# t0saki/YOLO-Infer-pt

Hardware: AMD Instinct MI355X
Metric: images/sec at 640x640 batch32, v11_n (forward + on-device NMS) (higher is better)
Workload: dtype bf16; 1 GPU; yolo_v11_n eval forward + NMS, 640x640, 32 images per GPU per step; per_gpu_batch=32, global_batch=32, image_size=640, parallelism=dp1, nms=on-device, conf 0.001, iou 0.65, max_det 300

## Files before the change

### yolo-infer-pt_amd/csrc/c3k2.hip

```cpp
#include "common.h"
#include "dtypes.h"

namespace yh {

namespace {

typedef float f32x16 __attribute__((ext_vector_type(16)));

template <typename T> struct CMfma;
template <> struct CMfma<__bf16> {
    static __device__ __forceinline__ f32x16 step(const uint4& a, const uint4& b, const f32x16& c) {
        return __builtin_amdgcn_mfma_f32_32x32x16_bf16(__builtin_bit_cast(bf16x8, a), __builtin_bit_cast(bf16x8, b), c, 0,
                                                       0, 0);
    }
};
template <> struct CMfma<_Float16> {
    static __device__ __forceinline__ f32x16 step(const uint4& a, const uint4& b, const f32x16& c) {
        return __builtin_amdgcn_mfma_f32_32x32x16_f16(__builtin_bit_cast(f16x8, a), __builtin_bit_cast(f16x8, b), c, 0, 0,
                                                      0);
    }
};

constexpr int NWV = CSP_THREADS / 64;

__device__ __forceinline__ void cs_glds(const void* src, unsigned lds_addr) {
#if defined(__HIP_DEVICE_COMPILE__)
    unsigned keep;
    asm volatile("s_mov_b32 %0, m0\n\ts_mov_b32 m0, %2\n\ts_nop 0\n\tglobal_load_lds_dwordx4 %1, off\n\ts_mov_b32 m0, %0"
                 : "=&s"(keep) : "v"(src), "s"(lds_addr) : "memory");
#else
    (void)src; (void)lds_addr;
#endif
}
__device__ __forceinline__ void cs_barrier() { asm volatile("s_waitcnt lgkmcnt(0)\n\ts_barrier" ::: "memory"); }

__device__ __forceinline__ void cs_wait_vm(int n) {
    if (n >= 8) asm volatile("s_waitcnt vmcnt(8)" ::: "memory");
    else if (n >= 4) asm volatile("s_waitcnt vmcnt(4)" ::: "memory");
    else if (n >= 2) asm volatile("s_waitcnt vmcnt(2)" ::: "memory");
    else asm volatile("s_waitcnt vmcnt(0)" ::: "memory");
}

#ifdef YH_CSP_TRACE
constexpr int CS_TR = 12, CS_TR_TILES = 16, CS_TR_WG = 256, CS_TR_OPS = 4;
__device__ unsigned long long csp_trace_buf[CS_TR_OPS * CS_TR_WG * CS_TR_TILES * CS_TR];
#define CS_STAMP(k) do { if (trp) trp[k] = __builtin_amdgcn_s_memtime(); } while (0)
#else
#define CS_STAMP(k) do { } while (0)
#endif

__device__ __forceinline__ uint4 cs_rd(unsigned addr) {
#if defined(__HIP_DEVICE_COMPILE__)
    typedef __attribute__((address_space(3))) const uint4* lp;
    return *reinterpret_cast<lp>((size_t)addr);
#else
    (void)addr;
    return uint4{};
#endif
}
__device__ __forceinline__ void cs_wr(unsigned addr, uint4 v) {
#if defined(__HIP_DEVICE_COMPILE__)
    typedef __attribute__((address_space(3))) uint4* lp;
    *reinterpret_cast<lp>((size_t)addr) = v;
#else
    (void)addr; (void)v;
#endif
}
__device__ __forceinline__ float4 cs_rdf(unsigned addr) {
    const uint4 u = cs_rd(addr);
    return make_float4(__uint_as_float(u.x), __uint_as_float(u.y), __uint_as_float(u.z), __uint_as_float(u.w));
}

struct CsLayout {
    int w1, w2, w3, w4, b1, b2, b3, b4, prm;
};
__host__ __device__ constexpr CsLayout cs_layout(int ni, int nc, int no) {
    const int nh = (nc + 1) / 2, na3 = (nc + 1) / 2;
    CsLayout L{};
    L.w1 = 0;
    L.w2 = L.w1 + nc * ni * 1024;
    L.w3 = L.w2 + 9 * nc * 1024;
    L.w4 = L.w3 + na3 * 9 * nh * 1024;
    L.b1 = L.w4 + no * 3 * nc * 1024;
    L.b2 = L.b1 + 32 * nc * 4;
    L.b3 = L.b2 + 32 * 4;
    L.b4 = L.b3 + 32 * na3 * 4;
    L.prm = (L.b4 + 32 * no * 4 + 1023) & ~1023;
    return L;
}
struct CsTile {
    int lx, lt, lr, lc, total;
};
__host__ __device__ inline CsTile cs_tile(int TH, int TW, int ni, int nc, int no) {
    const int nh = (nc + 1) / 2;
    const CsLayout L = cs_layout(ni, nc, no);
    const int XP = (TH + 4) * (TW + 4), MP = (TH + 2) * (TW + 2), NP = TH * TW;
    CsTile t{};
    t.lx = L.prm;
    t.lt = t.lx + (ni ? ((XP * (16 * ni + 8) * 2 + 1023) & ~1023) : 0);
    t.lr = t.lt + XP * (32 * nc + 8) * 2;
    t.lc = t.lr + MP * (16 * nh + 8) * 2;
    t.total = t.lc + NP * (16 * nc + 8) * 2;
    return t;
}

template <typename T>
__device__ __forceinline__ void cs_act(const f32x16& acc, unsigned bias_addr, uint4 (&o)[2]) {
    float v[16];
#pragma unroll
    for (int q = 0; q < 4; ++q) {
        const float4 b = cs_rdf(bias_addr + 16 * q);
        v[4 * q] = acc[4 * q] + b.x;
        v[4 * q + 1] = acc[4 * q + 1] + b.y;
        v[4 * q + 2] = acc[4 * q + 2] + b.z;
        v[4 * q + 3] = acc[4 * q + 3] + b.w;
    }
    T t[16];
#pragma unroll
    for (int i = 0; i < 16; ++i) t[i] = fromf<T>(silu<T>(v[i]));
    o[0] = *reinterpret_cast<const uint4*>(&t[0]);
    o[1] = *reinterpret_cast<const uint4*>(&t[8]);
}

template <typename T>
__device__ __forceinline__ uint4 cs_act_half(const f32x16& acc, unsigned bias_addr, int hh) {
#if defined(__HIP_DEVICE_COMPILE__)
    float v[8];
#pragma unroll
    for (int e = 0; e < 8; ++e)
        v[e] = __uint_as_float(
            __builtin_amdgcn_permlane32_swap(__float_as_uint(acc[e]), __float_as_uint(acc[8 + e]), false, false)[0]);
    const float4 b0 = cs_rdf(bias_addr + 32 * hh), b1 = cs_rdf(bias_addr + 32 * hh + 16);
    v[0] += b0.x; v[1] += b0.y; v[2] += b0.z; v[3] += b0.w;
    v[4] += b1.x; v[5] += b1.y; v[6] += b1.z; v[7] += b1.w;
    T t[8];
#pragma unroll
    for (int i = 0; i < 8; ++i) {
        float p = silu<T>(v[i]);
        asm("" : "+v"(p));
        t[i] = fromf<T>(p);
    }
    return *reinterpret_cast<const uint4*>(&t[0]);
#else
    (void)acc; (void)bias_addr; (void)hh;
    return uint4{};
#endif
}

template <typename T, int NA, int NK, typename BAddr, typename Epi>
__device__ __forceinline__ void cs_phase(unsigned aimg, int npx, BAddr baddr, Epi epi) {
    const int lane = threadIdx.x & 63, wv = threadIdx.x >> 6, l32 = lane & 31;
    const int items = NA * ((npx + 31) >> 5);
    for (int i0 = wv; i0 < items; i0 += 2 * NWV) {
        const int i1 = i0 + NWV;
        const int a0 = i0 % NA, a1 = i1 % NA;
        const int p0 = (i0 / NA) * 32 + l32, p1 = (i1 / NA) * 32 + l32;
        const int c0 = p0 < npx ? p0 : npx - 1, c1 = p1 < npx ? p1 : npx - 1;
        const unsigned ai0 = aimg + (unsigned)(a0 * NK * 1024 + lane * 16);
        const unsigned ai1 = aimg + (unsigned)(a1 * NK * 1024 + lane * 16);
        f32x16 acc0, acc1;
#pragma unroll
        for (int e = 0; e < 16; ++e) { acc0[e] = 0.f; acc1[e] = 0.f; }
        if (i1 < items) {
#pragma unroll
            for (int k = 0; k < NK; ++k) {
                const uint4 f0 = cs_rd(ai0 + k * 1024), f1 = NA > 1 ? cs_rd(ai1 + k * 1024) : f0;
                const uint4 x0 = cs_rd(baddr(c0, k)), x1 = cs_rd(baddr(c1, k));
                acc0 = CMfma<T>::step(f0, x0, acc0);
                acc1 = CMfma<T>::step(f1, x1, acc1);
            }
            if (p0 < npx) epi(a0, p0, acc0);
            if (p1 < npx) epi(a1, p1, acc1);
        } else {
#pragma unroll
            for (int k = 0; k < NK; ++k) acc0 = CMfma<T>::step(cs_rd(ai0 + k * 1024), cs_rd(baddr(c0, k)), acc0);
            if (p0 < npx) epi(a0, p0, acc0);
        }
    }
}

#ifdef YH_CSP_TRACE
constexpr int cs_trace_op(int ni, int, int no) { return ni == 2 ? 0 : ni == 4 ? 1 : no == 2 ? 2 : 3; }
#endif

template <typename T, int NI, int NC, int NO>
__global__ __launch_bounds__(CSP_THREADS) void csp_fused(const CspArgs A) {
    constexpr int NH = (NC + 1) / 2, NA3 = (NC + 1) / 2;
    constexpr int SX = 16 * NI + 8, ST = 32 * NC + 8, SR = 16 * NH + 8, SC = 16 * NC + 8;
    constexpr CsLayout L = cs_layout(NI, NC, NO);
    extern __shared__ __attribute__((aligned(16))) char sm[];
    typedef __attribute__((address_space(3))) char* lds_c;
    const unsigned lds0 = (unsigned)(size_t)(lds_c)sm;
    const int TH = A.TH, TW = A.TW, XW = TW + 4, MW = TW + 2;
    const int XP = (TH + 4) * XW, MP = (TH + 2) * MW, NP = TH * TW;
    const CsTile G = cs_tile(TH, TW, NI, NC, NO);
    const unsigned LX = lds0 + G.lx, LT = lds0 + G.lt, LR = lds0 + G.lr, LC = lds0 + G.lc;
    const int lane = threadIdx.x & 63, hh = lane >> 5;
    const int wvu = __builtin_amdgcn_readfirstlane(threadIdx.x >> 6);
    const T* x = reinterpret_cast<const T*>(A.x);
    T* y = reinterpret_cast<T*>(A.y);

    {
        const char* prm = reinterpret_cast<const char*>(A.prm);
        for (int i0 = wvu * 64; i0 < L.prm / 16; i0 += CSP_THREADS) cs_glds(prm + (size_t)(i0 + lane) * 16, lds0 + i0 * 16);
    }
    constexpr bool TAIL = NI == 0;
    constexpr int NCH = TAIL ? 4 * NC : 2 * NI;
    constexpr int CPX = NCH + 1;
    const unsigned LD = TAIL ? LT : LX;
    auto load_x = [&](int t) {
        const int n = t / A.tiles, tix = t - n * A.tiles;
        const int ty = tix / A.ntw, tx = tix - ty * A.ntw;
        const int h0 = ty * TH - 2, w0 = tx * TW - 2;
        const int total = XP * CPX;
        for (int i0 = wvu * 64; i0 < total; i0 += CSP_THREADS) {
            const int q = i0 + lane;
            const int px = q / CPX, c = q - px * CPX;
            const int r = px / XW, cc = px - r * XW;
            const int gh = h0 + r, gw = w0 + cc;
            const bool ok = q < total && c < NCH && (unsigned)gh < (unsigned)A.H && (unsigned)gw < (unsigned)A.W;
            const void* src = ok ? (const void*)(x + (((long long)n * A.H + gh) * A.W + gw) * A.ldx + c * 8) : A.zero;
            cs_glds(src, LD + i0 * 16);
        }
    };
    const int t0 = xcd_remap(blockIdx.x, gridDim.x);
    if (t0 < A.ntiles) load_x(t0);

    const int p4_items = NO * ((NP + 31) >> 5);
    const int p4_stores = wvu < p4_items ? 2 * ((p4_items - wvu + NWV - 1) / NWV) : 0;
    int young = 0;
#ifdef YH_CSP_TRACE
    int trk = 0;
#endif
    for (int t = t0; t < A.ntiles; t += gridDim.x) {
        const int n = t / A.tiles, tix = t - n * A.tiles;
        const int ty = tix / A.ntw, tx = tix - ty * A.ntw;
        const int h0 = ty * TH, w0 = tx * TW;
#ifdef YH_CSP_TRACE
        unsigned long long* trp = nullptr;
        if (threadIdx.x == 0 && blockIdx.x < CS_TR_WG && trk < CS_TR_TILES) {
            trp = csp_trace_buf + ((size_t)(cs_trace_op(NI, NC, NO) * CS_TR_WG + blockIdx.x) * CS_TR_TILES + trk) * CS_TR;
            trp[10] = __builtin_amdgcn_s_memrealtime();
            trp[11] = (unsigned long long)TH | (unsigned long long)TW << 16 | (unsigned long long)(t + 1) << 32;
        }
        ++trk;
#endif
        CS_STAMP(0);
        cs_wait_vm(young);
        CS_STAMP(1);
        cs_barrier();
        CS_STAMP(2);

        if constexpr (!TAIL) {
        cs_phase<T, NC, NI>(
                lds0 + L.w1, XP,
                [&](int px, int k) { return LX + (unsigned)(px * SX + 16 * k + 8 * hh) * 2; },
                [&](int a, int px, const f32x16& acc) {
                    uint4 o[2];
                    cs_act<T>(acc, lds0 + L.b1 + (32 * a + 16 * hh) * 4, o);
                    const int r = px / XW, cc = px - r * XW;
                    const int gh = h0 - 2 + r, gw = w0 - 2 + cc;
                    if (!((unsigned)gh < (unsigned)A.H && (unsigned)gw < (unsigned)A.W)) o[0] = o[1] = make_uint4(0, 0, 0, 0);
                    const unsigned d = LT + (unsigned)(px * ST + 32 * a + 16 * hh) * 2;
                    cs_wr(d, o[0]);
                    cs_wr(d + 16, o[1]);
                });
        CS_STAMP(3);
        cs_barrier();
        CS_STAMP(4);
        if (t + (int)gridDim.x < A.ntiles) load_x(t + gridDim.x);
        }

        cs_phase<T, 1, 9 * NC>(
            lds0 + L.w2, MP,
            [&](int px, int k) {
                const int cb = k / 9, tap = k - 9 * (k / 9), kh = tap / 3, kw = tap - 3 * (tap / 3);
                const int r = px / MW, cc = px - r * MW;
                return LT + (unsigned)(((r + kh) * XW + cc + kw) * ST + 16 * NC + 16 * cb + 8 * hh) * 2;
            },
            [&](int, int px, const f32x16& acc) {
                if constexpr (NH == 1) {
                    uint4 o = cs_act_half<T>(acc, lds0 + L.b2, hh);
                    const int r = px / MW, cc = px - r * MW;
                    const int gh = h0 - 1 + r, gw = w0 - 1 + cc;
                    if (!((unsigned)gh < (unsigned)A.H && (unsigned)gw < (unsigned)A.W)) o = make_uint4(0, 0, 0, 0);
                    cs_wr(LR + (unsigned)(px * SR + 8 * hh) * 2, o);
                    return;
                }
                if (16 * hh >= 16 * NH) return;
                uint4 o[2];
                cs_act<T>(acc, lds0 + L.b2 + 16 * hh * 4, o);
                const int r = px / MW, cc = px - r * MW;
                const int gh = h0 - 1 + r, gw = w0 - 1 + cc;
                if (!((unsigned)gh < (unsigned)A.H && (unsigned)gw < (unsigned)A.W)) o[0] = o[1] = make_uint4(0, 0, 0, 0);
                const unsigned d = LR + (unsigned)(px * SR + 16 * hh) * 2;
                cs_wr(d, o[0]);
                cs_wr(d + 16, o[1]);
            });
        CS_STAMP(5);
        cs_barrier();
        CS_STAMP(6);

        cs_phase<T, NA3, 9 * NH>(
                lds0 + L.w3, NP,
                [&](int px, int k) {
                    const int cb = k / 9, tap = k - 9 * (k / 9), kh = tap / 3, kw = tap - 3 * (tap / 3);
                    const int r = px / TW, cc = px - r * TW;
                    return LR + (unsigned)(((r + kh) * MW + cc + kw) * SR + 16 * cb + 8 * hh) * 2;
                },
                [&](int a, int px, const f32x16& acc) {
                    if constexpr (NC == 1) {
                        const uint4 o = cs_act_half<T>(acc, lds0 + L.b3, hh);
                        const int r = px / TW, cc = px - r * TW;
                        const uint4 rv = cs_rd(LT + (unsigned)(((r + 2) * XW + cc + 2) * ST + 16 * NC + 8 * hh) * 2);
                        const T* ov = reinterpret_cast<const T*>(&o);
                        const T* rr = reinterpret_cast<const T*>(&rv);
                        T s[8];
#pragma unroll
                        for (int e = 0; e < 8; ++e) s[e] = fromf<T>(tof(ov[e]) + tof(rr[e]));
                        cs_wr(LC + (unsigned)(px * SC + 8 * hh) * 2, *reinterpret_cast<const uint4*>(s));
                        return;
                    }
                    const int co = 32 * a + 16 * hh;
                    if (co >= 16 * NC) return;
                    uint4 o[2];
                    cs_act<T>(acc, lds0 + L.b3 + co * 4, o);
                    const int r = px / TW, cc = px - r * TW;
                    const unsigned rs = LT + (unsigned)(((r + 2) * XW + cc + 2) * ST + 16 * NC + co) * 2;
#pragma unroll
                    for (int hf = 0; hf < 2; ++hf) {
                        const uint4 rv = cs_rd(rs + 16 * hf);
                        const T* ov = reinterpret_cast<const T*>(&o[hf]);
                        const T* rr = reinterpret_cast<const T*>(&rv);
                        T s[8];
#pragma unroll
                        for (int e = 0; e < 8; ++e) s[e] = fromf<T>(tof(ov[e]) + tof(rr[e]));
                        o[hf] = *reinterpret_cast<const uint4*>(s);
                    }
                    const unsigned d = LC + (unsigned)(px * SC + co) * 2;
                    cs_wr(d, o[0]);
                    cs_wr(d + 16, o[1]);
                });
        CS_STAMP(7);
        cs_barrier();
        CS_STAMP(8);

        cs_phase<T, NO, 3 * NC>(
                lds0 + L.w4, NP,
                [&](int px, int k) {
                    const int r = px / TW, cc = px - r * TW;
                    return k < 2 * NC ? LT + (unsigned)(((r + 2) * XW + cc + 2) * ST + 16 * k + 8 * hh) * 2
                                      : LC + (unsigned)(px * SC + 16 * (k - 2 * NC) + 8 * hh) * 2;
                },
                [&](int a, int px, const f32x16& acc) {
                    uint4 o[2];
                    const int co = 32 * a + 16 * hh;
                    cs_act<T>(acc, lds0 + L.b4 + co * 4, o);
                    const int r = px / TW, cc = px - r * TW;
                    const int gh = h0 + r, gw = w0 + cc;
                    if ((unsigned)gh < (unsigned)A.H && (unsigned)gw < (unsigned)A.W) {
                        uint4* d = reinterpret_cast<uint4*>(y + (((long long)n * A.H + gh) * A.W + gw) * A.ldy + co);
                        d[0] = o[0];
                        d[1] = o[1];
                    }
                });
        CS_STAMP(9);
        if constexpr (!TAIL) young = h0 + TH <= A.H && w0 + TW <= A.W ? p4_stores : 0;
        if constexpr (TAIL) {
            cs_barrier();
            if (t + (int)gridDim.x < A.ntiles) load_x(t + gridDim.x);
        }
    }
    asm volatile("s_waitcnt vmcnt(0)" ::: "memory");
}

#define YH_CSP_LIST(X) X(2, 1, 2) X(4, 2, 4) X(0, 2, 2) X(0, 2, 4)

template <typename T>
int launch_csp_t(const CspArgs& a, int grid, hipStream_t s) {
    const int lds = csp_lds(a.TH, a.TW, a.ni, a.nc, a.no);
    if (lds == 0 || grid <= 0 || a.ldx % 8 || a.ldy % 8) return (int)hipErrorInvalidValue;
#define YH_CSP_CASE(NI, NC, NO)                                                                              \
    if (a.ni == NI && a.nc == NC && a.no == NO) {                                                            \
        static bool attr = false;                                                                            \
        if (!attr) {                                                                                         \
            (void)hipFuncSetAttribute(reinterpret_cast<const void*>(&csp_fused<T, NI, NC, NO>),              \
                                      hipFuncAttributeMaxDynamicSharedMemorySize, 160 * 1024);               \
            attr = true;                                                                                     \
        }                                                                                                    \
        hipLaunchKernelGGL((csp_fused<T, NI, NC, NO>), dim3((unsigned)grid), dim3(CSP_THREADS), lds, s, a); \
        return (int)hipGetLastError();                                                                       \
    }
    YH_CSP_LIST(YH_CSP_CASE)
#undef YH_CSP_CASE
    return (int)hipErrorInvalidValue;
}

}

int csp_prm_bytes(int ni, int nc, int no) { return cs_layout(ni, nc, no).prm; }

void csp_offsets(int ni, int nc, int no, int (&off)[9]) {
    const CsLayout L = cs_layout(ni, nc, no);
    const int v[9] = {L.w1, L.w2, L.w3, L.w4, L.b1, L.b2, L.b3, L.b4, L.prm};
    for (int i = 0; i < 9; ++i) off[i] = v[i];
}

int csp_lds(int TH, int TW, int ni, int nc, int no) {
    bool inst = false;
#define YH_CSP_HAS(NI, NC, NO) inst = inst || (ni == NI && nc == NC && no == NO);
    YH_CSP_LIST(YH_CSP_HAS)
#undef YH_CSP_HAS
    if (!inst || TH < 1 || TW < 1) return 0;
    const int b = cs_tile(TH, TW, ni, nc, no).total;
    return b <= 160 * 1024 ? b : 0;
}

#ifdef YH_CSP_TRACE
extern "C" int yh_debug_csp_trace(unsigned long long* dst, int n) {
    if (n > CS_TR_OPS * CS_TR_WG * CS_TR_TILES * CS_TR) n = CS_TR_OPS * CS_TR_WG * CS_TR_TILES * CS_TR;
    return (int)hipMemcpyFromSymbol(dst, HIP_SYMBOL(csp_trace_buf), (size_t)n * 8, 0, hipMemcpyDeviceToHost);
}
#endif

int launch_csp(int dtype, const CspArgs& a, int grid, hipStream_t s) {
    switch (dtype) {
        case F16: return launch_csp_t<_Float16>(a, grid, s);
        case BF16: return launch_csp_t<__bf16>(a, grid, s);
    }
    return (int)hipErrorInvalidValue;
}

}
```

### yolo-infer-pt_amd/csrc/common.h

```cpp
#pragma once
#include <hip/hip_runtime.h>
#include <stdint.h>

namespace yh {

enum DType { F32 = 0, F16 = 1, BF16 = 2 };
inline int dtype_size(int dt) { return dt == F32 ? 4 : 2; }

enum Act { ACT_ID = 0, ACT_SILU = 1 };

struct ConvArgs {
    const void* in0; int ldc0, c0, up0, h0, w0;
    const void* in1; int ldc1, c1, up1, h1, w1;
    int Hi, Wi, Ho, Wo, stride, pad, KH, KW, Cin, K, Kp, M;
    const void* w;
    const float* bias;
    const int* ktab;
    void* out; int ldo;
    const void* res; int ldr;
    int Cout;
    int act;
    int gm, gn;
    const void* zero;
    int ks;
};

struct FirstConvArgs {
    const void* const* io;
    int H, W, Ho, Wo, Cout, ldo, M;
    const float* w;
    const float* bias;
    void* out;
    int act;
    int in_u8;
};

struct Stem2Args {
    const void* const* io;
    int H, W, Hs, Ws, Ho, Wo, B;
    const float* b1;
    int c1, c2;
    const void* prm;
// ... 96 lines not shown
    int B, H, W;
    const void* prm;
    int hh;
    int bands;
    int nbuf;
    unsigned long long* trace;
};
int c3k_prm_bytes(int hh);
void c3k_offsets(int hh, int (&off)[9]);
int c3k_lds(int H, int W, int hh);
int c3k_bands(int B, int H, int W, int hh);
int c3k_region_px(int H, int W, int bands);
int launch_c3k(int dtype, const C3kArgs& a, hipStream_t s);

struct BoxDflLevel {
    const void* x; int ldx;
    int H, W; float stride; int aoff;
    const void* w; int wld; const float* b;
    int wg0;
};
struct BoxDflArgs {
    BoxDflLevel lv[3];
    int nlv, B, nk, nc, A;
    const void* const* io;
    int tpw;
};
struct CspArgs {
    const void* x; int ldx;
    void* y; int ldy;
    int H, W, B;
    const void* prm;
    int ni, nc, no;
    int TH, TW, ntw, tiles, ntiles;
    const void* zero;
};
#ifndef YH_CSP_THREADS
#define YH_CSP_THREADS 1024
#endif
constexpr int CSP_THREADS = YH_CSP_THREADS;
int csp_prm_bytes(int ni, int nc, int no);
void csp_offsets(int ni, int nc, int no, int (&off)[9]);
int csp_lds(int TH, int TW, int ni, int nc, int no);
int launch_csp(int dtype, const CspArgs& a, int grid, hipStream_t s);

constexpr int BOX_DFL_TPW = 2;
int launch_box_dfl(int dtype, const BoxDflArgs& a, hipStream_t s);

struct BoxChainLevel {
    const void* x; int ldx, C0;
    int H, W;
    int TH, TW, ntw, tiles;
    int nkc;
    float stride; int aoff;
    const void* prm;
    int wg0;
};
struct BoxChainArgs {
    BoxChainLevel lv[3];
    int nlv, B, nc, A;
    const void* const* io;
    const void* zero;
};
int bx_prm_bytes(int C0);
bool bx_ok(int C0);
bool bx_tile(int H, int W, int& TH, int& TW);
int launch_box_chain(int dtype, const BoxChainArgs& a, hipStream_t s);

constexpr int PWC_THREADS = 512;
constexpr int PWC_MAX_STAGES = 6, PWC_MAX_RUNS = 4, PWC_MAX_LOADS = 6;
struct PwcRun {
    int lds;
    int ld;
    int nkb;
};
struct PwcStage {
    int K, N, act, nrun;
// ... 41 lines not shown
```

### yolo-infer-pt_amd/csrc/engine.cpp

```cpp
#include <hip/hip_runtime.h>

#include <algorithm>
#include <cmath>
#include <cstdio>
#include <cstring>
#include <map>
#include <memory>
#include <stdexcept>
#include <string>
#include <vector>

#include "common.h"
#include "conv_mx.h"
#include "match_host.h"
#include "merge_host.h"
#include "yolo_hip.h"


namespace yh {

static thread_local std::string g_err;

struct Fail : std::runtime_error {
    int code;
// ... 673 lines not shown
                        const float v = d.wf[((size_t)co * d.cin + ch) * 9 + tap];
                        dst[((size_t)(a * nk + k) * 64 + lane) * 8 + j] = dtype == BF16 ? f2bf(v) : f2h(v);
                    }
        float* bd = reinterpret_cast<float*>(img.data() + bias_off);
        for (int i = 0; i < d.cout; ++i) bd[i] = d.bf[i];
        void* dev = nullptr;
        HIPCHECK(hipMalloc(&dev, img.size()));
        HIPCHECK(hipMemcpy(dev, img.data(), img.size(), hipMemcpyHostToDevice));
        d.mx_w.emplace("stem2", dev);
        d1.mx_w.emplace("stem2_dep", nullptr);
        return dev;
    }
    bool fuse_csp(const std::vector<Seg>& in, const std::vector<int>& logical, int c, int out_ch, View out) const {
        if (dtype == F32 || !opt.fuse) return false;
        if (in.size() != 1 || in[0].up || in[0].v.C != logical[0] || logical[0] % 16 || c % 16 || out_ch % 32) return false;
        if (out.coff % 8 || in[0].v.coff % 8) return false;
        int TH, TW;
        return csp_tile(logical[0] / 16, c / 16, out_ch / 32, 1, 1 << 30, 1 << 30, 1, TH, TW);
    }
    bool fuse_csp_tail(int c, int out_ch, View out) const {
        if (dtype == F32 || !opt.fuse) return false;
        if (c % 16 || out_ch % 32 || out.coff % 8) return false;
        int TH, TW;
        return csp_tile(0, c / 16, out_ch / 32, 1, 1 << 30, 1 << 30, 1, TH, TW);
    }
    bool tail_first() const { return opt.csp_tail; }
    static int csp_items(int TH, int TW, int ni, int nc, int no) {
        const auto nb = [](int px) { return (px + 31) / 32; };
        return (ni ? nc * nb((TH + 4) * (TW + 4)) : 0) + nb((TH + 2) * (TW + 2)) + ((nc + 1) / 2 + no) * nb(TH * TW);
    }
    static bool csp_tile(int ni, int nc, int no, int B, int H, int W, int cus, int& TH, int& TW) {
        if (const char* e = getenv("YH_CSP_TILE")) {
            int th = 0, tw = 0;
            if (sscanf(e, "%dx%d", &th, &tw) == 2 && th > 0 && tw > 0 && th <= H && tw <= W &&
                csp_lds(th, tw, ni, nc, no) > 0) {
                TH = th;
                TW = tw;
                return true;
            }
        }
        if (CSP_THREADS >= 1024) {
            constexpr long long CSP_TILE_FIXED = 7400, CSP_TILE_ITEM = 230;
            long long best = -1;
            H = std::min(H, 1 << 12);
            W = std::min(W, 1 << 12);
            for (int th : {2, 4, 8, 10, 12, 16}) {
                if (th > H || (th == 2 && H >= 4)) continue;
                for (int tw = 4; tw <= W; tw += 4) {
                    if (csp_lds(th, tw, ni, nc, no) <= 0) break;
                    const long long nt = (long long)B * ((H + th - 1) / th) * ((W + tw - 1) / tw);
                    const long long cost = ((nt + cus - 1) / cus) * (CSP_TILE_FIXED + CSP_TILE_ITEM * csp_items(th, tw, ni, nc, no));
                    if (best < 0 || cost < best) {
                        best = cost;
                        TH = th;
                        TW = tw;
                    }
                    if (nt <= cus) break;
                }
            }
            return best >= 0;
        }
        static const int cand[][2] = {{8, 16}, {8, 8}, {4, 16}, {4, 8}, {2, 8}, {2, 4}};
        for (int lim : {80 * 1024, 160 * 1024})
            for (auto& c : cand) {
                if (c[0] > H || c[1] > W || (lim == 80 * 1024 && c[0] * c[1] < 64)) continue;
                const int b = csp_lds(c[0], c[1], ni, nc, no);
                if (b > 0 && b <= lim) {
                    TH = c[0];
                    TW = c[1];
                    return true;
                }
            }
        return false;
    }
    const void* csp_params(const Op& op) {
// ... 826 lines not shown
                const ConvDesc& d = convs[op.conv];
                Stem2Args a{};
                a.io = (const void* const*)io_dev;
                a.H = H; a.W = W; a.Hs = H >> 1; a.Ws = W >> 1; a.Ho = H >> 2; a.Wo = W >> 2; a.B = B;
                a.b1 = d.b_dev;
                a.c1 = d.cout; a.c2 = convs[op.cs[0]].cout;
                a.prm = stem2_params(op, a.prm_bias, a.prm_stem);
                a.out = ptr(op.out);
                a.ldo = ldc(op.out);
                a.in_u8 = in_u8;
                stem2_tiles(a.Ho, a.Wo, a.ntw, a.nth);
                rc = launch_stem2(dtype, a, s);
                break;
            }
            case OP_CSP: {
                CspArgs a{};
                const View& xv = op.in[0].v;
                const int lv = tensors[xv.t].level;
                a.x = ptr(xv);
                a.ldx = ldc(xv);
                a.y = ptr(op.out);
                a.ldy = ldc(op.out);
                a.H = H >> lv;
                a.W = W >> lv;
                a.B = B;
                a.prm = csp_params(op);
                a.ni = op.cs[0] >= 0 ? convs[op.cs[0]].cin / 16 : 0;
                a.nc = convs[op.cs[1]].cin / 16;
                a.no = convs[op.cs[3]].cout / 32;
                if (!num_cus) HIPCHECK(hipDeviceGetAttribute(&num_cus, hipDeviceAttributeMultiprocessorCount, device));
                require(csp_tile(a.ni, a.nc, a.no, B, a.H, a.W, num_cus, a.TH, a.TW), op.label + ": no LDS tile");
                csp_plan[{GraphKey{B, H, W}, (int)oi}] = "c3k2_t" + std::to_string(a.TH) + "x" + std::to_string(a.TW);
                a.ntw = (a.W + a.TW - 1) / a.TW;
                a.tiles = a.ntw * ((a.H + a.TH - 1) / a.TH);
                a.ntiles = B * a.tiles;
                a.zero = zero_dev;
                {
                    const int lds = csp_lds(a.TH, a.TW, a.ni, a.nc, a.no);
                    const int per_cu = CSP_THREADS < 1024 && lds > 0 && lds <= 80 * 1024 ? 2 : 1;
                    rc = launch_csp(dtype, a, std::min(a.ntiles, per_cu * num_cus), s);
                }
                break;
            }
            case OP_C3K: {
                C3kArgs a{};
                const View& xv = op.in[0].v;
                const int lv = tensors[xv.t].level;
                a.x = ptr(xv);
                a.ldx = ldc(xv);
                a.y = ptr(op.out);
                a.ldy = ldc(op.out);
                a.H = H >> lv;
                a.W = W >> lv;
                a.B = B;
                a.prm = c3k_params(op);
                a.hh = convs[op.ck[0]].cout;
                rc = launch_c3k(dtype, a, s);
                break;
            }
        }
        if (rc != 0) throw Fail(YH_EHIP, "launch of " + op.label + " failed: " + hipGetErrorString((hipError_t)rc));
    }

    void free_plans() {
        plans.clear();
        cur_plan = nullptr;
    }
// ... 873 lines not shown
```

### yolo-infer-pt_amd/csrc/head.hip

```cpp
#include "common.h"
#include "dtypes.h"

namespace yh {

namespace {

typedef float f32x16 __attribute__((ext_vector_type(16)));
typedef float f32x2 __attribute__((ext_vector_type(2)));

template <typename T> struct HMfma;
template <> struct HMfma<__bf16> {
    static __device__ __forceinline__ f32x16 step(const uint4& a, const uint4& b, const f32x16& c) {
        return __builtin_amdgcn_mfma_f32_32x32x16_bf16(__builtin_bit_cast(bf16x8, a), __builtin_bit_cast(bf16x8, b), c, 0,
                                                       0, 0);
    }
};
template <> struct HMfma<_Float16> {
    static __device__ __forceinline__ f32x16 step(const uint4& a, const uint4& b, const f32x16& c) {
        return __builtin_amdgcn_mfma_f32_32x32x16_f16(__builtin_bit_cast(f16x8, a), __builtin_bit_cast(f16x8, b), c, 0, 0,
                                                      0);
    }
};

constexpr int NWV = HEAD_CLS_THREADS / 64;
// ... 28 lines not shown
    do {                \
    } while (0)
#endif
constexpr int HC_CK = 64;
#ifndef YH_HC_RB
#define YH_HC_RB 4
#endif
constexpr int HC_RB = YH_HC_RB;

struct HcLayout {
    int SX, SD, SM, r1, x2, prm, total;
};
__host__ __device__ inline HcLayout hc_layout(int TH, int TW, int C0, int c3) {
    HcLayout L;
    const int ck = C0 < HC_CK ? C0 : HC_CK;
    L.SX = ck + 8; L.SD = C0 + 8; L.SM = c3 + 8;
    const int MP = (TH + 2) * (TW + 2), NO = TH * TW;
    const int x = ((TH + 4) * (TW + 4) * L.SX * 2 + 1023) & ~1023;
    const int p1 = MP * L.SM * 2, p2 = NO * L.SM * 2;
    const int d1 = MP * L.SD * 2, d2 = NO * L.SM * 2;
    int a = x > p1 ? x : p1;
    a = a > p2 ? a : p2;
    L.r1 = (a + 15) & ~15;
    L.prm = L.r1 + (((d1 > d2 ? d1 : d2) + 15) & ~15);
    L.x2 = 0;
    if (C0 > HC_CK) {
        L.x2 = L.prm;
        L.prm += x;
    }
    L.total = L.prm + (((10 * C0 + 10 * c3 + 3 * 96) * 4 + 1023) & ~1023);
    return L;
}

struct HcDiv {
    unsigned m;
    int s;
};
__device__ __forceinline__ HcDiv hc_div(int d, int s) { return HcDiv{(1u << s) / (unsigned)d + 1u, s}; }
__device__ __forceinline__ int hc_q(int n, HcDiv f) { return (int)(((unsigned)n * f.m) >> f.s); }

template <typename T>
__device__ __forceinline__ void hc_dw(const T* src, int SW, int ss, T* dst, int DH, int DW, int ds, int c_lo, int C,
                                      const float* w, int wld, const float* b) {
    const int nrb = (DH + HC_RB - 1) / HC_RB, per_g = DW * nrb, ng = C >> 2;
    const HcDiv dw = hc_div(DW, 16);
    const int rs = SW * ss;
    float4 wt[9], bb;
    int wg = -1;
    auto load_w = [&](int g) {
        const int c0 = c_lo + g * 4;
#pragma unroll
        for (int k = 0; k < 9; ++k) wt[k] = *reinterpret_cast<const float4*>(w + k * wld + c0);
        bb = *reinterpret_cast<const float4*>(b + c0);
        wg = g;
    };
    hc_barrier();
    const HcDiv dn = hc_div(ng, 24);
    if ((int)threadIdx.x < ng * per_g) load_w((int)threadIdx.x - hc_q(threadIdx.x, dn) * ng);
    for (int q = threadIdx.x; q < ng * per_g; q += HEAD_CLS_THREADS) {
        const int p = hc_q(q, dn), g = q - p * ng;
        const int rb = hc_q(p, dw), c = p - rb * DW;
        const int r0 = rb * HC_RB, c0 = c_lo + g * 4;
        if (g != wg) load_w(g);
        const T* sp = src + (r0 * SW + c) * ss + g * 4;
        const int lim = DH + 1 - r0, lim_off = lim * rs;
        uint2 xv[HC_RB + 2][3];
#pragma unroll
        for (int r = 0; r < HC_RB + 2; ++r) {
            const int ro = r <= lim ? r * rs : lim_off;
#pragma unroll
            for (int kw = 0; kw < 3; ++kw) xv[r][kw] = *reinterpret_cast<const uint2*>(sp + ro + kw * ss);
        }
// ... 498 lines not shown
```

Baseline: 41830 images/s.

## Cut integer index arithmetic in fused C3k2 kernel with magic division and precomputed offsets

Replaces per-pixel integer divisions in the fused CSP kernel with 24-bit multiply-shift reciprocals, precomputes per-thread load offsets for input tile staging, and hoists row base addresses for the 3x3 tap loops so each k step is one add. Tile coordinates are advanced incrementally instead of being re-divided each iteration, and the first MFMA uses a zero constant instead of zero-initialising the accumulators. Validity checks are added so the 32-bit offset math is only used when its preconditions hold. The tile cost-model constants are also retuned, which can change the chosen tile sizes.

```diff
diff --git a/yolo-infer-pt_amd/csrc/c3k2.hip b/yolo-infer-pt_amd/csrc/c3k2.hip
--- a/yolo-infer-pt_amd/csrc/c3k2.hip
+++ b/yolo-infer-pt_amd/csrc/c3k2.hip
@@ -49,10 +49,12 @@
 #define CS_STAMP(k) do { } while (0)
 #endif
 
+typedef unsigned u32x4 __attribute__((ext_vector_type(4)));
 __device__ __forceinline__ uint4 cs_rd(unsigned addr) {
 #if defined(__HIP_DEVICE_COMPILE__)
-    typedef __attribute__((address_space(3))) const uint4* lp;
-    return *reinterpret_cast<lp>((size_t)addr);
+    typedef __attribute__((address_space(3))) const u32x4* lp;
+    const u32x4 v = *reinterpret_cast<lp>((size_t)addr);
+    return make_uint4(v[0], v[1], v[2], v[3]);
 #else
     (void)addr;
     return uint4{};
@@ -60,11 +62,16 @@
 }
 __device__ __forceinline__ void cs_wr(unsigned addr, uint4 v) {
 #if defined(__HIP_DEVICE_COMPILE__)
-    typedef __attribute__((address_space(3))) uint4* lp;
-    *reinterpret_cast<lp>((size_t)addr) = v;
+    typedef __attribute__((address_space(3))) u32x4* lp;
+    *reinterpret_cast<lp>((size_t)addr) = u32x4{v.x, v.y, v.z, v.w};
 #else
     (void)addr; (void)v;
 #endif
+}
+template <int S>
+__device__ __forceinline__ unsigned cs_px(unsigned px) {
+    static_assert(S % 8 == 0, "pixel strides are whole 16-byte chunks");
+    return __umul24(px, S / 8) << 4;
 }
 __device__ __forceinline__ float4 cs_rdf(unsigned addr) {
     const uint4 u = cs_rd(addr);
@@ -104,6 +111,15 @@
     return t;
 }
 
+constexpr int CS_DIV_S = 20;
+__host__ __device__ constexpr int cs_maxr(int ni) { return ni ? 4 : 6; }
+inline bool cs_index_ok(int TH, int TW, int ni, int nc) {
+    const long long XW = TW + 4, MW = TW + 2, XP = (TH + 4) * XW, MP = (TH + 2) * MW, NP = (long long)TH * TW;
+    const long long chunks = XP * ((ni ? 2 * ni : 4 * nc) + 1);
+    return TH + 4 < 0xffff && XW < 0xffff && chunks <= (long long)cs_maxr(ni) * CSP_THREADS &&
+           hc_exact(XP - 1, XW, CS_DIV_S) && hc_exact(MP - 1, MW, CS_DIV_S) && hc_exact(NP - 1, TW, CS_DIV_S);
+}
+
 template <typename T>
 __device__ __forceinline__ void cs_act(const f32x16& acc, unsigned bias_addr, uint4 (&o)[2]) {
     float v[16];
@@ -147,34 +163,44 @@
 #endif
 }
 
-template <typename T, int NA, int NK, typename BAddr, typename Epi>
-__device__ __forceinline__ void cs_phase(unsigned aimg, int npx, BAddr baddr, Epi epi) {
-    const int lane = threadIdx.x & 63, wv = threadIdx.x >> 6, l32 = lane & 31;
+struct CsB {
+    unsigned b[3];
+};
+template <typename T, int NA, int NK, typename Prep, typename BAddr, typename Epi>
+__device__ __forceinline__ void cs_phase(unsigned aimg, int npx, HcDiv dv, int RW, Prep prep, BAddr baddr, Epi epi) {
+    const int lane = threadIdx.x & 63, wv = __builtin_amdgcn_readfirstlane(threadIdx.x >> 6), l32 = lane & 31;
     const int items = NA * ((npx + 31) >> 5);
+    f32x16 zero;
+#pragma unroll
+    for (int e = 0; e < 16; ++e) zero[e] = 0.f;
     for (int i0 = wv; i0 < items; i0 += 2 * NWV) {
         const int i1 = i0 + NWV;
         const int a0 = i0 % NA, a1 = i1 % NA;
         const int p0 = (i0 / NA) * 32 + l32, p1 = (i1 / NA) * 32 + l32;
         const int c0 = p0 < npx ? p0 : npx - 1, c1 = p1 < npx ? p1 : npx - 1;
+        const int r0 = hc_q24(c0, dv), cc0 = c0 - (int)__umul24(r0, RW);
+        const CsB B0 = prep(c0, r0, cc0);
         const unsigned ai0 = aimg + (unsigned)(a0 * NK * 1024 + lane * 16);
-        const unsigned ai1 = aimg + (unsigned)(a1 * NK * 1024 + lane * 16);
-        f32x16 acc0, acc1;
-#pragma unroll
-        for (int e = 0; e < 16; ++e) { acc0[e] = 0.f; acc1[e] = 0.f; }
         if (i1 < items) {
+            const int r1 = hc_q24(c1, dv), cc1 = c1 - (int)__umul24(r1, RW);
+            const CsB B1 = prep(c1, r1, cc1);
+            const unsigned ai1 = aimg + (unsigned)(a1 * NK * 1024 + lane * 16);
+            f32x16 acc0, acc1;
 #pragma unroll
             for (int k = 0; k < NK; ++k) {
                 const uint4 f0 = cs_rd(ai0 + k * 1024), f1 = NA > 1 ? cs_rd(ai1 + k * 1024) : f0;
-                const uint4 x0 = cs_rd(baddr(c0, k)), x1 = cs_rd(baddr(c1, k));
-                acc0 = CMfma<T>::step(f0, x0, acc0);
-                acc1 = CMfma<T>::step(f1, x1, acc1);
+                const uint4 x0 = cs_rd(baddr(B0, k)), x1 = cs_rd(baddr(B1, k));
+                acc0 = CMfma<T>::step(f0, x0, k ? acc0 : zero);
+                acc1 = CMfma<T>::step(f1, x1, k ? acc1 : zero);
             }
-            if (p0 < npx) epi(a0, p0, acc0);
-            if (p1 < npx) epi(a1, p1, acc1);
+            if (p0 < npx) epi(a0, p0, r0, cc0, acc0);
+            if (p1 < npx) epi(a1, p1, r1, cc1, acc1);
         } else {
-#pragma unroll
-            for (int k = 0; k < NK; ++k) acc0 = CMfma<T>::step(cs_rd(ai0 + k * 1024), cs_rd(baddr(c0, k)), acc0);
-            if (p0 < npx) epi(a0, p0, acc0);
+            f32x16 acc0;
+#pragma unroll
+            for (int k = 0; k < NK; ++k)
+                acc0 = CMfma<T>::step(cs_rd(ai0 + k * 1024), cs_rd(baddr(B0, k)), k ? acc0 : zero);
+            if (p0 < npx) epi(a0, p0, r0, cc0, acc0);
         }
     }
 }
@@ -208,23 +234,40 @@
     constexpr int NCH = TAIL ? 4 * NC : 2 * NI;
     constexpr int CPX = NCH + 1;
     const unsigned LD = TAIL ? LT : LX;
-    auto load_x = [&](int t) {
-        const int n = t / A.tiles, tix = t - n * A.tiles;
-        const int ty = tix / A.ntw, tx = tix - ty * A.ntw;
+    const HcDiv dxw = hc_div(XW, CS_DIV_S), dmw = hc_div(MW, CS_DIV_S), dtw = hc_div(TW, CS_DIV_S);
+    constexpr int MAXR = cs_maxr(NI);
+    const int total = XP * CPX;
+    unsigned d_off[MAXR], d_rc[MAXR];
+#pragma unroll
+    for (int j = 0; j < MAXR; ++j) {
+        const int q = j * CSP_THREADS + (int)threadIdx.x;
+        const int px = q / CPX, c = q - px * CPX;
+        const int pc = px < XP ? px : XP - 1;
+        const int r = hc_q24(pc, dxw), cc = pc - (int)__umul24(r, XW);
+        d_rc[j] = q < total && c < NCH ? (unsigned)r | (unsigned)cc << 16 : 0xffffu;
+        d_off[j] = (__umul24(__umul24(r, A.W) + cc, A.ldx) + c * 8) * 2u;
+    }
+    auto load_x = [&](int n, int ty, int tx) {
         const int h0 = ty * TH - 2, w0 = tx * TW - 2;
-        const int total = XP * CPX;
-        for (int i0 = wvu * 64; i0 < total; i0 += CSP_THREADS) {
-            const int q = i0 + lane;
-            const int px = q / CPX, c = q - px * CPX;
-            const int r = px / XW, cc = px - r * XW;
-            const int gh = h0 + r, gw = w0 + cc;
-            const bool ok = q < total && c < NCH && (unsigned)gh < (unsigned)A.H && (unsigned)gw < (unsigned)A.W;
-            const void* src = ok ? (const void*)(x + (((long long)n * A.H + gh) * A.W + gw) * A.ldx + c * 8) : A.zero;
-            cs_glds(src, LD + i0 * 16);
+        const char* base = reinterpret_cast<const char*>(x + (((long long)n * A.H + h0) * A.W + w0) * A.ldx);
+        const unsigned rlo = h0 < 0 ? -h0 : 0, clo = w0 < 0 ? -w0 : 0;
+        const unsigned rn = min(TH + 4, A.H - h0) - rlo, cn = min(XW, A.W - w0) - clo;
+#pragma unroll
+        for (int j = 0; j < MAXR; ++j) {
+            const int i0 = j * CSP_THREADS + wvu * 64;
+            if (i0 < total) {
+                const unsigned r = d_rc[j] & 0xffffu, cc = d_rc[j] >> 16;
+                const bool ok = r - rlo < rn && cc - clo < cn;
+                const void* src = ok ? (const void*)(base + d_off[j]) : A.zero;
+                cs_glds(src, LD + i0 * 16);
+            }
         }
     };
     const int t0 = xcd_remap(blockIdx.x, gridDim.x);
-    if (t0 < A.ntiles) load_x(t0);
+    const int NG = gridDim.x;
+    const int gn = NG / A.tiles, gty = (NG - gn * A.tiles) / A.ntw, gtx = NG - gn * A.tiles - gty * A.ntw;
+    int n = t0 / A.tiles, ty = (t0 - n * A.tiles) / A.ntw, tx = t0 - n * A.tiles - ty * A.ntw;
+    if (t0 < A.ntiles) load_x(n, ty, tx);
 
     const int p4_items = NO * ((NP + 31) >> 5);
     const int p4_stores = wvu < p4_items ? 2 * ((p4_items - wvu + NWV - 1) / NWV) : 0;
@@ -232,10 +275,17 @@
 #ifdef YH_CSP_TRACE
     int trk = 0;
 #endif
-    for (int t = t0; t < A.ntiles; t += gridDim.x) {
-        const int n = t / A.tiles, tix = t - n * A.tiles;
-        const int ty = tix / A.ntw, tx = tix - ty * A.ntw;
+    for (int t = t0; t < A.ntiles; t += NG) {
         const int h0 = ty * TH, w0 = tx * TW;
+        int nn = n + gn, nty = ty + gty, ntx = tx + gtx;
+        if (ntx >= A.ntw) { ntx -= A.ntw; ++nty; }
+        if (nty >= A.nth) { nty -= A.nth; ++nn; }
+        const unsigned rlo2 = h0 < 2 ? 2 - h0 : 0, clo2 = w0 < 2 ? 2 - w0 : 0;
+        const unsigned rn2 = min(TH + 4, A.H - h0 + 2) - rlo2, cn2 = min(XW, A.W - w0 + 2) - clo2;
+        const unsigned rlo1 = h0 < 1 ? 1 : 0, clo1 = w0 < 1 ? 1 : 0;
+        const unsigned rn1 = min(TH + 2, A.H - h0 + 1) - rlo1, cn1 = min(MW, A.W - w0 + 1) - clo1;
+        const unsigned rn0 = min(TH, A.H - h0), cn0 = min(TW, A.W - w0);
+        char* ybase = reinterpret_cast<char*>(y + (((long long)n * A.H + h0) * A.W + w0) * A.ldy);
 #ifdef YH_CSP_TRACE
         unsigned long long* trp = nullptr;
         if (threadIdx.x == 0 && blockIdx.x < CS_TR_WG && trk < CS_TR_TILES) {
@@ -253,47 +303,47 @@
 
         if constexpr (!TAIL) {
         cs_phase<T, NC, NI>(
-                lds0 + L.w1, XP,
-                [&](int px, int k) { return LX + (unsigned)(px * SX + 16 * k + 8 * hh) * 2; },
-                [&](int a, int px, const f32x16& acc) {
+                lds0 + L.w1, XP, dxw, XW,
+                [&](int px, int, int) { return CsB{{LX + cs_px<SX>(px) + 16 * hh, 0, 0}}; },
+                [&](const CsB& B, int k) { return B.b[0] + 32 * k; },
+                [&](int a, int px, int r, int cc, const f32x16& acc) {
                     uint4 o[2];
                     cs_act<T>(acc, lds0 + L.b1 + (32 * a + 16 * hh) * 4, o);
-                    const int r = px / XW, cc = px - r * XW;
-                    const int gh = h0 - 2 + r, gw = w0 - 2 + cc;
-                    if (!((unsigned)gh < (unsigned)A.H && (unsigned)gw < (unsigned)A.W)) o[0] = o[1] = make_uint4(0, 0, 0, 0);
-                    const unsigned d = LT + (unsigned)(px * ST + 32 * a + 16 * hh) * 2;
+                    if (!((unsigned)r - rlo2 < rn2 && (unsigned)cc - clo2 < cn2)) o[0] = o[1] = make_uint4(0, 0, 0, 0);
+                    const unsigned d = LT + cs_px<ST>(px) + (32 * a + 16 * hh) * 2;
                     cs_wr(d, o[0]);
                     cs_wr(d + 16, o[1]);
                 });
         CS_STAMP(3);
         cs_barrier();
         CS_STAMP(4);
-        if (t + (int)gridDim.x < A.ntiles) load_x(t + gridDim.x);
+        if (t + NG < A.ntiles) load_x(nn, nty, ntx);
         }
 
         cs_phase<T, 1, 9 * NC>(
-            lds0 + L.w2, MP,
-            [&](int px, int k) {
+            lds0 + L.w2, MP, dmw, MW,
+            [&](int, int r, int cc) {
+                const unsigned b0 = LT + cs_px<ST>(__umul24(r, XW) + cc) + (16 * NC + 8 * hh) * 2;
+                const unsigned rs = cs_px<ST>(XW);
+                return CsB{{b0, b0 + rs, b0 + 2 * rs}};
+            },
+            [&](const CsB& B, int k) {
                 const int cb = k / 9, tap = k - 9 * (k / 9), kh = tap / 3, kw = tap - 3 * (tap / 3);
-                const int r = px / MW, cc = px - r * MW;
-                return LT + (unsigned)(((r + kh) * XW + cc + kw) * ST + 16 * NC + 16 * cb + 8 * hh) * 2;
+                return B.b[kh] + (kw * ST + 16 * cb) * 2;
             },
-            [&](int, int px, const f32x16& acc) {
+            [&](int, int px, int r, int cc, const f32x16& acc) {
+                const bool in = (unsigned)r - rlo1 < rn1 && (unsigned)cc - clo1 < cn1;
                 if constexpr (NH == 1) {
                     uint4 o = cs_act_half<T>(acc, lds0 + L.b2, hh);
-                    const int r = px / MW, cc = px - r * MW;
-                    const int gh = h0 - 1 + r, gw = w0 - 1 + cc;
-                    if (!((unsigned)gh < (unsigned)A.H && (unsigned)gw < (unsigned)A.W)) o = make_uint4(0, 0, 0, 0);
-                    cs_wr(LR + (unsigned)(px * SR + 8 * hh) * 2, o);
+                    if (!in) o = make_uint4(0, 0, 0, 0);
+                    cs_wr(LR + cs_px<SR>(px) + 16 * hh, o);
                     return;
                 }
                 if (16 * hh >= 16 * NH) return;
                 uint4 o[2];
                 cs_act<T>(acc, lds0 + L.b2 + 16 * hh * 4, o);
-                const int r = px / MW, cc = px - r * MW;
-                const int gh = h0 - 1 + r, gw = w0 - 1 + cc;
-                if (!((unsigned)gh < (unsigned)A.H && (unsigned)gw < (unsigned)A.W)) o[0] = o[1] = make_uint4(0, 0, 0, 0);
-                const unsigned d = LR + (unsigned)(px * SR + 16 * hh) * 2;
+                if (!in) o[0] = o[1] = make_uint4(0, 0, 0, 0);
+                const unsigned d = LR + cs_px<SR>(px) + 32 * hh;
                 cs_wr(d, o[0]);
                 cs_wr(d + 16, o[1]);
             });
@@ -302,31 +352,34 @@
         CS_STAMP(6);
 
         cs_phase<T, NA3, 9 * NH>(
-                lds0 + L.w3, NP,
-                [&](int px, int k) {
+                lds0 + L.w3, NP, dtw, TW,
+                [&](int, int r, int cc) {
+                    const unsigned b0 = LR + cs_px<SR>(__umul24(r, MW) + cc) + 16 * hh;
+                    const unsigned rs = cs_px<SR>(MW);
+                    return CsB{{b0, b0 + rs, b0 + 2 * rs}};
+                },
+                [&](const CsB& B, int k) {
                     const int cb = k / 9, tap = k - 9 * (k / 9), kh = tap / 3, kw = tap - 3 * (tap / 3);
-                    const int r = px / TW, cc = px - r * TW;
-                    return LR + (unsigned)(((r + kh) * MW + cc + kw) * SR + 16 * cb + 8 * hh) * 2;
+                    return B.b[kh] + (kw * SR + 16 * cb) * 2;
                 },
-                [&](int a, int px, const f32x16& acc) {
+                [&](int a, int px, int r, int cc, const f32x16& acc) {
+                    const unsigned tb = LT + cs_px<ST>(__umul24(r + 2, XW) + cc + 2) + 32 * NC;
                     if constexpr (NC == 1) {
                         const uint4 o = cs_act_half<T>(acc, lds0 + L.b3, hh);
-                        const int r = px / TW, cc = px - r * TW;
-                        const uint4 rv = cs_rd(LT + (unsigned)(((r + 2) * XW + cc + 2) * ST + 16 * NC + 8 * hh) * 2);
+                        const uint4 rv = cs_rd(tb + 16 * hh);
                         const T* ov = reinterpret_cast<const T*>(&o);
                         const T* rr = reinterpret_cast<const T*>(&rv);
                         T s[8];
 #pragma unroll
                         for (int e = 0; e < 8; ++e) s[e] = fromf<T>(tof(ov[e]) + tof(rr[e]));
-                        cs_wr(LC + (unsigned)(px * SC + 8 * hh) * 2, *reinterpret_cast<const uint4*>(s));
+                        cs_wr(LC + cs_px<SC>(px) + 16 * hh, *reinterpret_cast<const uint4*>(s));
                         return;
                     }
                     const int co = 32 * a + 16 * hh;
                     if (co >= 16 * NC) return;
                     uint4 o[2];
                     cs_act<T>(acc, lds0 + L.b3 + co * 4, o);
-                    const int r = px / TW, cc = px - r * TW;
-                    const unsigned rs = LT + (unsigned)(((r + 2) * XW + cc + 2) * ST + 16 * NC + co) * 2;
+                    const unsigned rs = tb + co * 2;
 #pragma unroll
                     for (int hf = 0; hf < 2; ++hf) {
                         const uint4 rv = cs_rd(rs + 16 * hf);
@@ -337,7 +390,7 @@
                         for (int e = 0; e < 8; ++e) s[e] = fromf<T>(tof(ov[e]) + tof(rr[e]));
                         o[hf] = *reinterpret_cast<const uint4*>(s);
                     }
-                    const unsigned d = LC + (unsigned)(px * SC + co) * 2;
+                    const unsigned d = LC + cs_px<SC>(px) + co * 2;
                     cs_wr(d, o[0]);
                     cs_wr(d + 16, o[1]);
                 });
@@ -346,20 +399,19 @@
         CS_STAMP(8);
 
         cs_phase<T, NO, 3 * NC>(
-                lds0 + L.w4, NP,
-                [&](int px, int k) {
-                    const int r = px / TW, cc = px - r * TW;
-                    return k < 2 * NC ? LT + (unsigned)(((r + 2) * XW + cc + 2) * ST + 16 * k + 8 * hh) * 2
-                                      : LC + (unsigned)(px * SC + 16 * (k - 2 * NC) + 8 * hh) * 2;
+                lds0 + L.w4, NP, dtw, TW,
+                [&](int px, int r, int cc) {
+                    return CsB{{LT + cs_px<ST>(__umul24(r + 2, XW) + cc + 2) + 16 * hh,
+                                LC + cs_px<SC>(px) + 16 * hh, 0}};
                 },
-                [&](int a, int px, const f32x16& acc) {
+                [&](const CsB& B, int k) { return k < 2 * NC ? B.b[0] + 32 * k : B.b[1] + 32 * (k - 2 * NC); },
+                [&](int a, int, int r, int cc, const f32x16& acc) {
                     uint4 o[2];
                     const int co = 32 * a + 16 * hh;
                     cs_act<T>(acc, lds0 + L.b4 + co * 4, o);
-                    const int r = px / TW, cc = px - r * TW;
-                    const int gh = h0 + r, gw = w0 + cc;
-                    if ((unsigned)gh < (unsigned)A.H && (unsigned)gw < (unsigned)A.W) {
-                        uint4* d = reinterpret_cast<uint4*>(y + (((long long)n * A.H + gh) * A.W + gw) * A.ldy + co);
+                    if ((unsigned)r < rn0 && (unsigned)cc < cn0) {
+                        const unsigned off = (__umul24(__umul24(r, A.W) + cc, A.ldy) + co) * 2u;
+                        uint4* d = reinterpret_cast<uint4*>(ybase + off);
                         d[0] = o[0];
                         d[1] = o[1];
                     }
@@ -368,8 +420,11 @@
         if constexpr (!TAIL) young = h0 + TH <= A.H && w0 + TW <= A.W ? p4_stores : 0;
         if constexpr (TAIL) {
             cs_barrier();
-            if (t + (int)gridDim.x < A.ntiles) load_x(t + gridDim.x);
+            if (t + NG < A.ntiles) load_x(nn, nty, ntx);
         }
+        n = nn;
+        ty = nty;
+        tx = ntx;
     }
     asm volatile("s_waitcnt vmcnt(0)" ::: "memory");
 }
@@ -380,6 +435,7 @@
 int launch_csp_t(const CspArgs& a, int grid, hipStream_t s) {
     const int lds = csp_lds(a.TH, a.TW, a.ni, a.nc, a.no);
     if (lds == 0 || grid <= 0 || a.ldx % 8 || a.ldy % 8) return (int)hipErrorInvalidValue;
+    if (!csp_span_ok(a.TH, a.TW, a.W, a.ldx, a.ldy) || a.nth * a.ntw != a.tiles) return (int)hipErrorInvalidValue;
 #define YH_CSP_CASE(NI, NC, NO)                                                                              \
     if (a.ni == NI && a.nc == NC && a.no == NO) {                                                            \
         static bool attr = false;                                                                            \
@@ -411,7 +467,8 @@
 #define YH_CSP_HAS(NI, NC, NO) inst = inst || (ni == NI && nc == NC && no == NO);
     YH_CSP_LIST(YH_CSP_HAS)
 #undef YH_CSP_HAS
-    if (!inst || TH < 1 || TW < 1) return 0;
+    if (!inst || TH < 1 || TW < 1 || TH > 4096 || TW > 4096) return 0;
+    if (!cs_index_ok(TH, TW, ni, nc)) return 0;
     const int b = cs_tile(TH, TW, ni, nc, no).total;
     return b <= 160 * 1024 ? b : 0;
 }
diff --git a/yolo-infer-pt_amd/csrc/common.h b/yolo-infer-pt_amd/csrc/common.h
--- a/yolo-infer-pt_amd/csrc/common.h
+++ b/yolo-infer-pt_amd/csrc/common.h
@@ -8,6 +8,19 @@
 inline int dtype_size(int dt) { return dt == F32 ? 4 : 2; }
 
 enum Act { ACT_ID = 0, ACT_SILU = 1 };
+
+struct HcDiv {
+    unsigned m;
+    int s;
+};
+__host__ __device__ __forceinline__ HcDiv hc_div(int d, int s) { return HcDiv{(1u << s) / (unsigned)d + 1u, s}; }
+__host__ __device__ __forceinline__ int hc_q(int n, HcDiv f) { return (int)(((unsigned)n * f.m) >> f.s); }
+__device__ __forceinline__ int hc_q24(int n, HcDiv f) { return (int)(__umul24((unsigned)n, f.m) >> f.s); }
+inline bool hc_exact(long long nmax, long long d, int s) {
+    if (d < 1 || nmax < 0 || s > 24) return false;
+    const long long m = (1ll << s) / d + 1;
+    return nmax * d < (1ll << s) && nmax * m < (1ll << 32) && nmax < (1 << 24) && m < (1 << 24);
+}
 
 struct ConvArgs {
     const void* in0; int ldc0, c0, up0, h0, w0;
@@ -170,6 +183,7 @@
     const void* prm;
     int ni, nc, no;
     int TH, TW, ntw, tiles, ntiles;
+    int nth;
     const void* zero;
 };
 #ifndef YH_CSP_THREADS
@@ -180,6 +194,10 @@
 void csp_offsets(int ni, int nc, int no, int (&off)[9]);
 int csp_lds(int TH, int TW, int ni, int nc, int no);
 int launch_csp(int dtype, const CspArgs& a, int grid, hipStream_t s);
+inline bool csp_span_ok(int TH, int TW, int W, int ldx, int ldy) {
+    const long long px = (long long)(TH + 4) * W + TW + 4, ld = ldx > ldy ? ldx : ldy;
+    return W > 0 && ld > 0 && W < (1 << 24) && ld < (1 << 24) && px < (1 << 24) && (px * ld + ld) * 2 < (1ll << 31);
+}
 
 constexpr int BOX_DFL_TPW = 2;
 int launch_box_dfl(int dtype, const BoxDflArgs& a, hipStream_t s);
diff --git a/yolo-infer-pt_amd/csrc/engine.cpp b/yolo-infer-pt_amd/csrc/engine.cpp
--- a/yolo-infer-pt_amd/csrc/engine.cpp
+++ b/yolo-infer-pt_amd/csrc/engine.cpp
@@ -729,15 +729,14 @@
     static bool csp_tile(int ni, int nc, int no, int B, int H, int W, int cus, int& TH, int& TW) {
         if (const char* e = getenv("YH_CSP_TILE")) {
             int th = 0, tw = 0;
-            if (sscanf(e, "%dx%d", &th, &tw) == 2 && th > 0 && tw > 0 && th <= H && tw <= W &&
-                csp_lds(th, tw, ni, nc, no) > 0) {
+            if (sscanf(e, "%dx%d", &th, &tw) == 2 && th > 0 && tw > 0 && csp_lds(th, tw, ni, nc, no) > 0) {
                 TH = th;
                 TW = tw;
                 return true;
             }
         }
         if (CSP_THREADS >= 1024) {
-            constexpr long long CSP_TILE_FIXED = 7400, CSP_TILE_ITEM = 230;
+            constexpr long long CSP_TILE_FIXED = 6000, CSP_TILE_ITEM = 165;
             long long best = -1;
             H = std::min(H, 1 << 12);
             W = std::min(W, 1 << 12);
@@ -1630,7 +1629,9 @@
                 require(csp_tile(a.ni, a.nc, a.no, B, a.H, a.W, num_cus, a.TH, a.TW), op.label + ": no LDS tile");
                 csp_plan[{GraphKey{B, H, W}, (int)oi}] = "c3k2_t" + std::to_string(a.TH) + "x" + std::to_string(a.TW);
                 a.ntw = (a.W + a.TW - 1) / a.TW;
-                a.tiles = a.ntw * ((a.H + a.TH - 1) / a.TH);
+                require(csp_span_ok(a.TH, a.TW, a.W, a.ldx, a.ldy), op.label + ": map too wide for 32-bit tile offsets");
+                a.nth = (a.H + a.TH - 1) / a.TH;
+                a.tiles = a.ntw * a.nth;
                 a.ntiles = B * a.tiles;
                 a.zero = zero_dev;
                 {
diff --git a/yolo-infer-pt_amd/csrc/head.hip b/yolo-infer-pt_amd/csrc/head.hip
--- a/yolo-infer-pt_amd/csrc/head.hip
+++ b/yolo-infer-pt_amd/csrc/head.hip
@@ -84,12 +84,6 @@
     return L;
 }
 
-struct HcDiv {
-    unsigned m;
-    int s;
-};
-__device__ __forceinline__ HcDiv hc_div(int d, int s) { return HcDiv{(1u << s) / (unsigned)d + 1u, s}; }
-__device__ __forceinline__ int hc_q(int n, HcDiv f) { return (int)(((unsigned)n * f.m) >> f.s); }
 
 template <typename T>
 __device__ __forceinline__ void hc_dw(const T* src, int SW, int ss, T* dst, int DH, int DW, int ds, int c_lo, int C,
```

Result: faster. 43650 images/s (median of 6 runs) (+4.3%).
